# ut-amrl/nautilus

Measured on AMD Instinct MI355X. Metric: loop-closure candidate pairs/sec (1081-beam), higher is better.
Workload: dtype u16

## Files before the change

### nautilus_amd/csm.py

```python
import ctypes as C
import math

import numpy as np

from . import _lib
from ._lib import GridSpec, GridLayout, Search, Match, check, ptr

MATCH_DTYPE = np.dtype([("itheta", "<i4"), ("ix", "<i4"), ("iy", "<i4"), ("score", "<f4")])
assert MATCH_DTYPE.itemsize == C.sizeof(Match) == 16


def grid_spec(range_m=30.0, res=0.05, sigma=2.0, floor_p=1e-10, max_shift=40, cell_bits=16, skip_map=False, no_image=False):
    return GridSpec(float(range_m), float(res), float(sigma), float(floor_p), int(max_shift), int(cell_bits),
                    (_lib.NHIP_GRID_SKIP_MAP if skip_map else 0) | (_lib.NHIP_GRID_NO_IMAGE if no_image else 0), 0)


def search_spec(n_theta=61, nx=81, ny=81, theta_step=math.radians(1.0), exhaustive=False, dense=False, short_scans=False,
                exact_score=False, latency=False):
    flags = (_lib.NHIP_SEARCH_EXHAUSTIVE if exhaustive else 0) | (_lib.NHIP_SEARCH_DENSE if dense else 0) | \
            (_lib.NHIP_SEARCH_SHORT_SCANS if short_scans else 0) | (_lib.NHIP_SEARCH_EXACT_SCORE if exact_score else 0) | \
            (_lib.NHIP_SEARCH_LATENCY if latency else 0)
    return Search(int(n_theta), int(nx), int(ny), flags, float(theta_step))


# ... 175 lines not shown


def gate_floor(spec, min_score, n_points):
    out = C.c_int32(0)
    check(_lib.load().nhip_csm_gate_floor(C.byref(spec), float(min_score), int(n_points), C.byref(out)))
    return out.value


def bnb_stats():
    a, b = C.c_uint64(0), C.c_uint64(0)
    check(_lib.load().nhip_bnb_stats(C.byref(a), C.byref(b)))
    return a.value, b.value


def bnb_stats_levels():
    v = (C.c_uint64 * 24)()
    check(_lib.load().nhip_bnb_stats_levels(v))
    return {"blocks_whole": v[0], "blocks_total": v[1], "candidates_refined": v[2], "sub_blocks": v[3],
            "clk_wave_phase3": v[4], "clk_origins": v[5], "clk_sub_bounds": v[6], "clk_exact": v[7],
            "clk_slowest_wave": v[8], "clk_seeds": v[9], "clk_bounds": v[10], "clk_wave_phase3_100MHz": v[11],
            "pairs_handed_over": v[12], "clk_wave_second_kernel": v[13], "pose_evals16": v[14],
            "pairs_settled_by_gate": v[15], "passes_l2_runs": v[16], "passes_per_cell_field": v[17],
            "passes_per_cell_capacity": v[18], "edge_blocks_refined": v[19], "sub_blocks_without_pose": v[20],
            "edge_blocks_whole": v[21]}


def score_volume(scans, grids, src, slot, theta0, search, origin=(0, 0)):
    out = np.zeros((search.n_theta, search.nx, search.ny), dtype=np.int32)
    check(_lib.load().nhip_csm_scores(scans._h, grids._h, int(src), int(slot), float(theta0),
                                      int(origin[0]), int(origin[1]), C.byref(search), ptr(out)))
    return out


def match_to_transform(m, spec, search, theta0, origin=(0, 0)):
    tx = (origin[0] + int(m["ix"]) - (search.nx - 1) // 2) * spec.res
    ty = (origin[1] + int(m["iy"]) - (search.ny - 1) // 2) * spec.res
    th = theta0 + (int(m["itheta"]) - (search.n_theta - 1) // 2) * search.theta_step
    return np.float32(tx), np.float32(ty), np.float32(th)


class CorrelativeScanMatcher:

    def __init__(self, scanner_range, trans_range, low_res, high_res, sigma=2.0, cell_bits=16):
        self.params = _lib.CsmParams(float(scanner_range), float(trans_range), float(low_res), float(high_res),
                                     float(sigma), 1e-10, int(cell_bits), 0)

    def GetTransformation(self, pointcloud_a, pointcloud_b, rotation_a, rotation_b, rotation_restriction):
        a = np.ascontiguousarray(pointcloud_a, dtype=np.float32).reshape(-1, 2)
        b = np.ascontiguousarray(pointcloud_b, dtype=np.float32).reshape(-1, 2)
        score, tx, ty, th = C.c_double(0), C.c_float(0), C.c_float(0), C.c_float(0)
        check(_lib.load().nhip_csm_get_transformation(C.byref(self.params), ptr(a), len(a), ptr(b), len(b),
                                                      float(rotation_a), float(rotation_b), float(rotation_restriction),
                                                      C.byref(score), C.byref(tx), C.byref(ty), C.byref(th)))
        return score.value, ((np.float32(tx.value), np.float32(ty.value)), np.float32(th.value))


def last_launch():
    out = (C.c_int32 * 8)()
    check(_lib.load().nhip_csm_last_launch(out))
    form = {0: "fused", 1: "split, one round", 2: "split, rounds on one stream", 3: "split, rounds overlapped on the helper stream"}
    return {"form": form.get(out[0], "?"), "form_id": out[0], "pairs_per_round": out[1], "rounds_of_state": out[2],
            "rounds": out[3], "short_scans": bool(out[4]), "hand_over_kernel": bool(out[5]), "instrumented": bool(out[6] & 1),
            "l2_runs": bool(out[6] & 2), "n_pairs": out[7]}


def drop_in_cache_stats():
    v = [C.c_int64(0) for _ in range(4)]
    check(_lib.load().nhip_csm_cache_stats(*[C.byref(x) for x in v]))
    return dict(zip(("entries", "bytes", "hits", "misses"), (x.value for x in v)))


def drop_in_cache_clear():
    check(_lib.load().nhip_csm_cache_clear())


def drop_in_cache_configure(max_bytes):
    check(_lib.load().nhip_csm_cache_configure(int(max_bytes)))
```

### nautilus_amd/csrc/nhip_bnb.hip

```cpp
#include <atomic>
#include <mutex>
#include <type_traits>
#include <vector>

#ifndef NHIP_BNB_INSTR
#define NHIP_BNB_INSTR 0
#endif
#if NHIP_BNB_INSTR
#define csm_bnb_kernel csm_bnb_kernel_instr
#define csm_bnb_rot_kernel csm_bnb_rot_kernel_instr
#define launchers_product launchers_instr
#define BNB_STATS(P) ((P).stats)
#define BNB_TIMELINE(P) ((P).timeline)
#else
#define BNB_STATS(P) (static_cast<unsigned long long *>(nullptr))
#define BNB_TIMELINE(P) (static_cast<unsigned long long *>(nullptr))
#endif

#include "nhip_bnb_params.h"
#include "nhip_bnb_wave.h"
#include "nhip_bnb_origin.h"
#include "nhip_bnb_bounds.h"
#include "nhip_bnb_exact.h"

namespace nhip {

namespace {

using namespace bnb;

constexpr int BNB_THREADS = 64 * BNB_WAVES;

constexpr int N_WORK = 7;
struct PairCtx {
  const uint8_t *grid;
  const float2 *pts;
  int32_t n_pts, cx, cy, pair;
};

template <int CB>
__device__ __forceinline__ void process_candidate(const BnbParams &P, const PairCtx &C, int32_t k, int32_t v, int lane,
                                                  unsigned long long *best, uint32_t (&n)[N_WORK]) {
  const int Y = v / NB, X = v - NB * Y;
  const int32_t vx = block_extent(P.nx, X), vy = block_extent(P.ny, Y);
  const bool edge = vx < BNB_B || vy < BNB_B;
  float cf, sf;
  rotation_k(P, C.pair, k, &cf, &sf);
  if (P.levels >= 2) {
    const __amdgpu_buffer_rsrc_t p4 = uniform_rsrc(C.grid + P.grid_bytes + P.skip_bytes + P.pool_bytes, P.pool4_bytes);
    uint32_t sb[4];
    sub_bounds(P, p4, C.pts, C.n_pts, cf, sf, C.cx, C.cy, Y, X, lane, CB == 1 ? 1u : 257u, sb);
    n[1]++;
    n[4] += edge ? 1u : 0u;
    const uint32_t bsum = best_sum<false>(best);
    int alive = 0;
#pragma unroll
    for (int q = 0; q < 4; q++) alive += (sub_valid(vy, vx, q >> 1, q & 1) && sb[q] != 0u && sb[q] >= bsum) ? 1 : 0;
    if (alive == 0) return;
    if (alive <= 2) {
      const __amdgpu_buffer_rsrc_t rsrc = uniform_rsrc(C.grid, P.grid_bytes + P.skip_bytes);
#pragma unroll 1
      for (int q = 0; q < 4; q++) {
        const uint32_t b = q == 0 ? sb[0] : (q == 1 ? sb[1] : (q == 2 ? sb[2] : sb[3]));
        if (!sub_valid(vy, vx, q >> 1, q & 1) || b == 0u || b < best_sum<false>(best)) continue;
        const unsigned long long key = eval_sub<CB>(P, rsrc, C.pts, C.n_pts, cf, sf, C.cx, C.cy, k, Y, X, q >> 1, q & 1, lane);
        wave_atomic_max(best, key, lane);
        n[2]++;
        n[5] += sub_valid(vy, vx, q >> 1, q & 1) ? 0u : 1u;
      }
      return;
    }
  }
  const unsigned long long key = eval_block<CB>(P, C.grid, C.pts, C.n_pts, cf, sf, C.cx, C.cy, k, Y, X, lane);
  wave_atomic_max(best, key, lane);
  n[0]++;
  n[6] += edge ? 1u : 0u;
}

template <int CB, bool GLOBAL>
__device__ __forceinline__ void process_candidate_c(const BnbParams &P, __amdgpu_buffer_rsrc_t rsrc, uint32_t pitch8,
                                                    __amdgpu_buffer_rsrc_t rsrc16, const uint32_t *org, int32_t nch,
                                                    int32_t n_pts, int32_t k, int32_t Y, int32_t X,
                                                    uint32_t sb0, uint32_t sb1, uint32_t sb2, uint32_t sb3, int lane,
                                                    unsigned long long *best, uint32_t &bcopy, uint32_t (&n)[N_WORK]) {
  const uint32_t bsum = best_sum_cached<GLOBAL>(best, bcopy);
  const int32_t vx = block_extent(P.nx, X), vy = block_extent(P.ny, Y);
  const bool edge = vx < BNB_B || vy < BNB_B;
  n[4] += edge ? 1u : 0u;
  const bool ok0 = sub_valid(vy, vx, 0, 0), ok1 = sub_valid(vy, vx, 0, 1), ok2 = sub_valid(vy, vx, 1, 0), ok3 = sub_valid(vy, vx, 1, 1);
  const int alive = (ok0 && sb0 != 0u && sb0 >= bsum) + (ok1 && sb1 != 0u && sb1 >= bsum) + (ok2 && sb2 != 0u && sb2 >= bsum) +
                    (ok3 && sb3 != 0u && sb3 >= bsum);
  if (alive == 0) return;
  constexpr int WHOLE_MIN = 3;
  if (alive >= WHOLE_MIN) {
    int dy, dx;
    const uint32_t total = block_sums8(rsrc, pitch8, (uint32_t)P.hi_copy_bytes, org, nch, Y, X, lane, &dy, &dx);
    const int32_t ix = BNB_B * X + dx, iy = BNB_B * Y + dy;
    if (CB == 1) {
      const unsigned long long key = best_key(P, k, ix, iy, total, 32);
      wave_atomic_max(best, key, lane);
      if (GLOBAL) bcopy = max(bcopy, (uint32_t)(key >> 32));
    } else {
      n[3] += refine16<GLOBAL>(P, rsrc16, org, nch, n_pts, k, ix, iy, total, true, lane, best, bcopy);
    }
    n[0]++;
    n[6] += __ballot(ix < P.nx && iy < P.ny) != ~0ull ? 1u : 0u;
    return;
  }
#pragma unroll 1
  for (int q = 0; q < 4; q++) {
    const uint32_t b = q == 0 ? sb0 : (q == 1 ? sb1 : (q == 2 ? sb2 : sb3));
    if (!sub_valid(vy, vx, q >> 1, q & 1) || b == 0u || b < best_sum_cached<GLOBAL>(best, bcopy)) continue;
    int dy, dx;
    const uint32_t total = sub_sums8(rsrc, pitch8, (uint32_t)P.hi_copy_bytes, org, nch, Y, X, q >> 1, q & 1, lane, &dy, &dx);
    const int32_t ix = BNB_B * X + BNB_B4 * (q & 1) + dx, iy = BNB_B * Y + BNB_B4 * (q >> 1) + dy;
    if (CB == 1) {
      const unsigned long long key = best_key(P, k, ix, iy, total, 8);
      wave_atomic_max(best, key, lane);
      if (GLOBAL) bcopy = max(bcopy, (uint32_t)(key >> 32));
    } else {
      n[3] += refine16<GLOBAL>(P, rsrc16, org, nch, n_pts, k, ix, iy, total, lane < 16, lane, best, bcopy);
    }
    n[2]++;
    n[5] += __ballot(ix < P.nx && iy < P.ny) == 0ull ? 1u : 0u;
  }
}

struct PhaseClocks {
  long long org, strip, eval;
  uint32_t run_passes, cell_passes_field, cell_passes_full;
};

__device__ __forceinline__ void flush_stats(unsigned long long *stats, const uint32_t *n, int32_t pair, const PhaseClocks *clk,
                                            const uint32_t *edge = nullptr) {
  if (n) {
    if (n[0]) atomicAdd(&stats[0], (unsigned long long)n[0]);
    if (n[1]) atomicAdd(&stats[2], (unsigned long long)n[1]);
    if (n[2]) atomicAdd(&stats[3], (unsigned long long)n[2]);
    if (n[3]) atomicAdd(&stats[14], (unsigned long long)n[3]);
    if (pair < BNB_STATS_PAIRS) atomicAdd(&stats[BNB_STATS_HEAD + pair], 4ull * n[0] + n[2]);
  }
  if (edge) {
    if (edge[0]) atomicAdd(&stats[19], (unsigned long long)edge[0]);
    if (edge[1]) atomicAdd(&stats[20], (unsigned long long)edge[1]);
    if (edge[2]) atomicAdd(&stats[21], (unsigned long long)edge[2]);
  }
  if (clk) {
    atomicAdd(&stats[5], (unsigned long long)clk->org);
    atomicAdd(&stats[6], (unsigned long long)clk->strip);
    atomicAdd(&stats[7], (unsigned long long)clk->eval);
    if (clk->run_passes) atomicAdd(&stats[16], (unsigned long long)clk->run_passes);
    if (clk->cell_passes_field) atomicAdd(&stats[17], (unsigned long long)clk->cell_passes_field);
    if (clk->cell_passes_full) atomicAdd(&stats[18], (unsigned long long)clk->cell_passes_full);
  }
}

template <int CB, bool GLOBAL, bool RUNS = false>
__device__ __forceinline__ void rotation_pass(const BnbParams &P, const PairCtx &C, int32_t k, uint32_t u0, uint32_t u1,
                                              unsigned long long m0, unsigned long long m1, int lane,
                                              unsigned long long *best, uint32_t *done, uint32_t *org,
                                              uint32_t (&n_work)[N_WORK], PhaseClocks &clk, uint32_t *runs = nullptr) {
  long long t_mark = 0;
  float cf, sf;
  rotation_k(P, C.pair, k, &cf, &sf);
  if (BNB_STATS(P)) t_mark = clock64();
  int32_t nrc = RUNS_NONE;
  const int32_t nch = cache_origins<RUNS>(P, C.pts, C.n_pts, cf, sf, C.cx, C.cy, lane, org, true, runs, RUNS && P.l2_runs != 0, &nrc);
  if (BNB_STATS(P)) clk.org += clock64() - t_mark;
  if (RUNS && BNB_STATS(P)) {
    clk.run_passes += nrc > 0 ? 1u : 0u;
    clk.cell_passes_field += nrc == RUNS_FIELD ? 1u : 0u;
    clk.cell_passes_full += nrc == RUNS_FULL ? 1u : 0u;
  }
  const __amdgpu_buffer_rsrc_t rsrc16 = CB == 1 ? uniform_rsrc(C.grid, P.grid_bytes + P.skip_bytes)
                                                : uniform_rsrc(C.grid + P.hi_offset + 2 * P.hi_copy_bytes, P.t16_bytes);
  const __amdgpu_buffer_rsrc_t rsrc = uniform_rsrc(C.grid + P.hi_offset, 2 * P.hi_copy_bytes);
  const uint32_t pitch8 = (uint32_t)P.hi_tpr;
  const __amdgpu_buffer_rsrc_t p4 = uniform_rsrc(C.grid + P.grid_bytes + P.skip_bytes + P.pool_bytes, P.pool4_bytes);
  while ((m0 | m1) != 0ull) {
    const int b0 = m0 ? (int)__builtin_ctzll(m0) : 64 + (int)__builtin_ctzll(m1);
    const int Y = b0 / NB, X0 = b0 - NB * Y;
    int len = 1;
    while (len < 3 && X0 + len < NB) {
      const int b = b0 + len;
      if (!(((b < 64 ? m0 >> b : m1 >> (b - 64)) & 1ull))) break;
      len++;
    }
    uint32_t sb[12];
    uint32_t bcopy = GLOBAL ? best_sum<true>(best) : 0u;
    if (P.levels >= 2) {
      if (BNB_STATS(P)) t_mark = clock64();
      if (RUNS && nrc > 0) strip_bounds_c<RunList<RUN_CHUNKS>>(P, p4, runs + lane, nrc, Y, X0, len, CB == 1 ? 1u : 257u, sb);
      else strip_bounds_c<CellList>(P, p4, org, nch, Y, X0, len, CB == 1 ? 1u : 257u, sb);
      if (BNB_STATS(P)) clk.strip += clock64() - t_mark;
      n_work[1] += (uint32_t)len;
    } else {
#pragma unroll
      for (int q = 0; q < 12; q++) sb[q] = 0xffffffffu;
    }
#pragma unroll 1
    for (int t = 0; t < len; t++) {
      const int b = b0 + t;
      if (b < 64) m0 &= ~(1ull << b);
      else m1 &= ~(1ull << (b - 64));
      const uint32_t ub = (uint32_t)__builtin_amdgcn_readlane((int)(b < 64 ? u0 : u1), b & 63);
      if (ub < best_sum_cached<GLOBAL>(best, bcopy)) continue;
      const uint32_t s0 = t == 0 ? sb[0] : (t == 1 ? sb[4] : sb[8]), s1 = t == 0 ? sb[1] : (t == 1 ? sb[5] : sb[9]);
      const uint32_t s2 = t == 0 ? sb[2] : (t == 1 ? sb[6] : sb[10]), s3 = t == 0 ? sb[3] : (t == 1 ? sb[7] : sb[11]);
      if (BNB_STATS(P)) t_mark = clock64();
      process_candidate_c<CB, GLOBAL>(P, rsrc, pitch8, rsrc16, org, nch, C.n_pts, k, Y, X0 + t, s0, s1, s2, s3, lane, best,
                                      bcopy, n_work);
      if (BNB_STATS(P)) clk.eval += clock64() - t_mark;
      if (done && wave_leader(lane)) done[b] = 0u;
    }
  }
}

__device__ __forceinline__ void read_entry(const RotEntry *ent, int32_t *pair, int32_t *k, unsigned long long *m0,
                                           unsigned long long *m1) {
  const unsigned long long w0 = ent->w[0], w1 = ent->w[1], w2 = ent->w[2], w3 = ent->w[3];
  *pair = (int32_t)(w0 >> 24);
  *k = (int32_t)(w0 & 0xffffffull);
  *m0 = w1 | (w2 << 41);
  *m1 = (w2 >> 23) | (w3 << 18);
}

__device__ __forceinline__ void pair_context(const BnbParams &P, int32_t pair, PairCtx *C) {
  const int32_t src = P.pair_src[pair], slot = P.pair_slot[pair];
  const int32_t beg = P.offsets[src];
  C->grid = P.grids + (size_t)slot * P.slot_bytes;
  C->pts = P.xy + beg;
  C->n_pts = P.offsets[src + 1] - beg;
  C->cx = P.pair_origin ? P.pair_origin[2 * pair] : 0;
  C->cy = P.pair_origin ? P.pair_origin[2 * pair + 1] : 0;
  C->pair = pair;
}
// ... 158 lines not shown
        u1 = s_U[k * 128 + 64 + lane];
        const uint32_t bsum = best_sum<false>(s_best);
        m0 = __ballot(u0 != 0u && u0 >= bsum);
        m1 = __ballot(u1 != 0u && u1 >= bsum && lane + 64 < NB * NB);
        if ((m0 | m1) == 0ull) continue;
        if (heavy && (uint32_t)rank >= P.keep_ranks) {
          const uint32_t lx = (xcd + (uint32_t)rank) & 7u;
          const uint32_t e = wave_fetch_add(P.rot_count + 8 * lx, 1u, lane);
          if (e < P.rot_cap) {
            if (lane < 4) {
              const unsigned long long M41 = (1ull << 41) - 1ull;
              const unsigned long long word = lane == 0   ? ((unsigned long long)(uint32_t)pair << 24) | (uint32_t)k
                                              : lane == 1 ? (m0 & M41)
                                              : lane == 2 ? ((m0 >> 41) | (m1 << 23)) & M41
                                                          : (m1 >> 18);
              P.rot_list[(size_t)lx * P.rot_cap + e].w[lane] = word;
            }
            handed_over = true;
            continue;
          }
        }
        have = true;
      }
      if (have) rotation_pass<CB, false>(P, C, k, u0, u1, m0, m1, lane, s_best, done, org, n_work, clk);
      if (state == SEED) {
        __syncthreads();
        if (BNB_TIMELINE(P) && threadIdx.x == 0 && pair < BNB_STATS_PAIRS) BNB_TIMELINE(P)[4 * pair + 2] = wall_clock64();
        if (BNB_STATS(P)) {
          t_busy = clock64();
          t_wall = wall_clock64();
        }
        for (int32_t kk = threadIdx.x; kk < P.n_theta; kk += THREADS) {
          const unsigned long long mine = s_kmax[kk];
          int32_t rank = 0;
          for (int32_t j = 0; j < P.n_theta; j++) rank += s_kmax[j] > mine ? 1 : 0;
          s_order[rank] = (uint32_t)kk;
        }
        if (P.rot_list || SPLIT) {
          const uint32_t bsum = best_sum<false>(s_best);
          uint32_t mine = 0u;
          for (int32_t kk = wave; kk < P.n_theta; kk += WAVES) {
            const uint32_t c0 = s_U[kk * 128 + lane], c1 = s_U[kk * 128 + 64 + lane];
            mine += (uint32_t)__builtin_popcountll(__ballot(c0 != 0u && c0 >= bsum)) +
                    (uint32_t)__builtin_popcountll(__ballot(c1 != 0u && c1 >= bsum && lane + 64 < NB * NB));
          }
          if (wave_leader(lane)) atomicAdd(s_qn, mine);
        }
// ... 93 lines not shown
    flush_stats(stats_g, nullptr, pair, nullptr, n_work + 4);
  }
  __syncthreads();
  if (threadIdx.x == 0) {
    P.keys[pair] = *s_best;
    if (BNB_TIMELINE(P) && pair < BNB_STATS_PAIRS) {
      uint32_t hw;
      asm volatile("s_getreg_b32 %0, hwreg(HW_REG_HW_ID)" : "=s"(hw));
      uint32_t xcc;
      asm volatile("s_getreg_b32 %0, hwreg(HW_REG_XCC_ID)" : "=s"(xcc));
      BNB_TIMELINE(P)[4 * pair + 3] = (wall_clock64() & 0xfffffffffffull) | ((unsigned long long)((hw >> 8) & 0xffu) << 44) |
                                      ((unsigned long long)(xcc & 0xfu) << 52);
    }
    if (BNB_STATS(P) && BY_ROT) atomicAdd(&BNB_STATS(P)[8], *s_slow);
    if (stats_g) {
      const uint32_t n_all[4] = {s_cnt[0], s_cnt[3], s_cnt[4], s_cnt[5]};
      flush_stats(stats_g, n_all, pair, nullptr);
      atomicAdd(&stats_g[1], (unsigned long long)(P.n_theta * P.nbx * P.nby));
    }
  }
}

template <int CB>
__global__ __launch_bounds__(256, 4) void csm_bnb_rot_kernel(BnbParams P) {
  const int lane = threadIdx.x & 63;
  const uint32_t xcd = blockIdx.x & 7u;
  const uint32_t filled = P.rot_count[8 * xcd];
  const uint32_t count = filled < P.rot_cap ? filled : P.rot_cap;
  const RotEntry *list = P.rot_list + (size_t)xcd * P.rot_cap;
  __shared__ uint32_t s_org2[4 * ORG_WAVE];
  __shared__ uint32_t s_run2[4 * RUN_WAVE];
  uint32_t *org = s_org2 + (threadIdx.x >> 6) * ORG_WAVE + lane;
  uint32_t *runs = s_run2 + (threadIdx.x >> 6) * RUN_WAVE;
  PhaseClocks clk = {0, 0, 0, 0u, 0u, 0u};
  const long long t0 = BNB_STATS(P) ? clock64() : 0;
  for (;;) {
    const uint32_t i = wave_fetch_add(P.rot_count + 8 * xcd + 1, 1u, lane);
    if (i >= count) break;
    int32_t pair, k;
    unsigned long long m0, m1;
    read_entry(list + i, &pair, &k, &m0, &m1);
    PairCtx C;
    pair_context(P, pair, &C);
    uint32_t n[N_WORK] = {};
    rotation_pass<CB, true, true>(P, C, k, 0xffffffffu, 0xffffffffu, m0, m1, lane, &P.keys[pair], nullptr, org, n, clk, runs);
    if (BNB_STATS(P) && lane == 0) flush_stats(BNB_STATS(P), n, pair, nullptr, n + 4);
  }
  if (BNB_STATS(P) && lane == 0) {
    atomicAdd(&BNB_STATS(P)[13], (unsigned long long)(clock64() - t0));
    flush_stats(BNB_STATS(P), nullptr, 0, &clk);
  }
}

constexpr int SORT_THREADS = 1024;
constexpr int SORT_BUCKETS = 16 * 21;
__device__ __forceinline__ int cand_bucket(uint32_t c) {
  if (c == 0u) return SORT_BUCKETS - 1;
  const int e = 31 - __builtin_clz(c);
  const int f = e >= 4 ? (int)((c >> (e - 4)) & 15u) : (int)((c << (4 - e)) & 15u);
  const int b = 16 * e + f;
  return b >= SORT_BUCKETS - 1 ? 0 : SORT_BUCKETS - 2 - b;
}
__device__ __forceinline__ uint32_t cand_shares(const BnbParams &P, uint32_t c) {
  const uint32_t w = 1u + c / P.split_min;
  return w < P.split_max ? w : P.split_max;
}

__global__ __launch_bounds__(SORT_THREADS) void csm_bnb_order_kernel(BnbParams P) {
// ... 94 lines not shown
  }
  __syncthreads();
  unsigned long long *best = shared ? &P.keys[pair] : &s_best2;
  uint32_t *next = shared ? &P.ps_next[pair] : &s_next2;
  const uint32_t *rows = P.ps_rows + (size_t)pair * (size_t)P.n_theta * 128u;
  uint32_t *org = s_org2 + (threadIdx.x >> 6) * ORG_WAVE + lane;
  uint32_t *runs = s_run2 + (threadIdx.x >> 6) * RUN_WAVE;
  PairCtx C;
  pair_context(P, pair, &C);
  uint32_t n_work[N_WORK] = {};
  PhaseClocks clk = {0, 0, 0, 0u, 0u, 0u};
  const long long t0 = BNB_STATS(P) ? clock64() : 0;
  for (;;) {
    const uint32_t rank = wave_fetch_add(next, 1u, lane);
    if (rank >= live) break;
    const uint32_t u0 = rows[(size_t)rank * 128u + lane], u1 = rows[(size_t)rank * 128u + 64 + lane];
    const uint32_t kmax = (uint32_t)__builtin_amdgcn_readlane((int)u1, 62);
    const int32_t k = __builtin_amdgcn_readlane((int)u1, 63);
    const uint32_t bsum = best_sum<true>(best);
    if (kmax < bsum) break;
    const unsigned long long m0 = __ballot(u0 != 0u && u0 >= bsum);
    const unsigned long long m1 = __ballot(u1 != 0u && u1 >= bsum && lane + 64 < NB * NB);
    if ((m0 | m1) == 0ull) continue;
    rotation_pass<CB, true, true>(P, C, k, u0, u1, m0, m1, lane, best, nullptr, org, n_work, clk, runs);
  }
  if (BNB_STATS(P) && lane == 0) {
    atomicAdd(&BNB_STATS(P)[13], (unsigned long long)(clock64() - t0));
    flush_stats(BNB_STATS(P), n_work, pair, &clk, n_work + 4);
  }
  if (BNB_TIMELINE(P) && lane == 0 && pair < BNB_STATS_PAIRS)
    atomicMax(&BNB_TIMELINE(P)[5 * (size_t)BNB_STATS_PAIRS + 2 + pair], wall_clock64());
  if (!shared) {
    __syncthreads();
    if (threadIdx.x == 0) P.keys[pair] = s_best2;
  }
}

}

namespace bnb {

namespace {
template <int CB, bool PL, bool BR, bool SP = false>
int launch_main(const BnbParams &P, const BnbPlan &plan, hipStream_t s) {
  constexpr int THREADS = SP ? 64 * SPLIT_WAVES : BNB_THREADS;
  const size_t lds = lds_bytes((size_t)plan.lds_first, P.n_theta, SP);
  const int64_t blocks = (int64_t)P.pairs_per_xcd * 8;
// ... 74 lines not shown
```

### nautilus_amd/csrc/nhip_bnb_exact.h

```cpp
#pragma once
#include "nhip_bnb_origin.h"

namespace nhip {
namespace {

constexpr int SEG_CHUNKS = 32;
constexpr int EVAL_CHUNKS = 2;

template <bool GLOBAL>
__device__ __forceinline__ uint32_t best_sum(unsigned long long *best) {
  unsigned long long b;
  if (GLOBAL) b = __hip_atomic_load(best, __ATOMIC_RELAXED, __HIP_MEMORY_SCOPE_AGENT);
  else b = *(volatile unsigned long long *)best;
  return (uint32_t)__builtin_amdgcn_readfirstlane((int)(uint32_t)(b >> 32));
}
template <bool GLOBAL>
__device__ __forceinline__ uint32_t best_sum_cached(unsigned long long *best, uint32_t copy) {
  return GLOBAL ? copy : best_sum<false>(best);
}

__device__ __forceinline__ unsigned long long best_key(const BnbParams &P, int32_t k, int32_t ix, int32_t iy, uint32_t total,
                                                       int top) {
  unsigned long long key = 0ull;
  if (ix < P.nx && iy < P.ny) {
// ... 351 lines not shown
    }
  }
  uint32_t R[32];
#pragma unroll
  for (int y = 0; y < 8; y++) {
    R[4 * y + 0] = E[y][0];
    R[4 * y + 1] = O[y][0] - ((E[y][0] >> 16) << 8);
    R[4 * y + 2] = E[y][1];
    R[4 * y + 3] = O[y][1] - ((E[y][1] >> 16) << 8);
  }
  rs_step<32, 1>(R, lane & 1);
  rs_step<16, 2>(R, lane & 2);
  rs_step<8, 4>(R, lane & 4);
  uint32_t V[8];
#pragma unroll
  for (int i = 0; i < 4; i++) {
    V[2 * i] = R[i] & 0xffffu;
    V[2 * i + 1] = R[i] >> 16;
  }
  rs_step<8, 8>(V, lane & 8);
  rs_step<4, 16>(V, lane & 16);
  rs_step<2, 32>(V, lane & 32);
  const int r = 8 * (2 * ((lane >> 5) & 1) + ((lane >> 4) & 1)) + 4 * ((lane >> 2) & 1) + 2 * ((lane >> 1) & 1) + (lane & 1);
  const int f = (lane >> 3) & 1, d = r & 3;
  *dy = r >> 2;
  *dx = 4 * (d >> 1) + (d & 1) + 2 * f;
  return V[0];
}

__device__ __forceinline__ uint32_t pose_sum16(const BnbParams &P, __amdgpu_buffer_rsrc_t rsrc16, const uint32_t *org,
                                               int32_t nch, int32_t ix, int32_t iy) {
  uint32_t acc = 0u;
#pragma unroll
  for (int c = 0; c < OCL; c++) {
    if (c >= nch) continue;
    const uint32_t o = origin_of(org, c);
    acc += org_cnt(o) * (uint32_t)__builtin_amdgcn_raw_buffer_load_b16(
                            rsrc16, (int)t16_tiled(org_row(o) + (uint32_t)iy, org_col(o) + (uint32_t)ix, (uint32_t)P.t16_tpr), 0, 0);
  }
  return wave_sum(acc);
}

template <bool GLOBAL>
__device__ __forceinline__ uint32_t refine16(const BnbParams &P, __amdgpu_buffer_rsrc_t rsrc16, const uint32_t *org,
                                             int32_t nch, int32_t n_pts, int32_t k, int32_t ix, int32_t iy, uint32_t hsum,
                                             bool mine, int lane, unsigned long long *best, uint32_t &bcopy) {
// ... 22 lines not shown
```

### nautilus_amd/csrc/nhip_bnb_host.hip

```cpp
#include <atomic>
#include <memory>
#include <mutex>
#include <vector>

#include "nhip_bnb_params.h"

namespace nhip {

using namespace bnb;

namespace {

size_t bnb_lds_first(const GridLayout &L, bool pool_lds) {
  const size_t pool = pool_lds ? (size_t)L.pool_bytes : 0;
  return pool > (size_t)ORG_LDS ? pool : (size_t)ORG_LDS;
}
size_t bnb_lds_bytes(const GridLayout &L, const nhip_search_t *search, bool pool_lds) {
  return lds_bytes(bnb_lds_first(L, pool_lds), search->n_theta, false);
}
constexpr size_t LDS_MAX = 160 * 1024;

struct TimerScope {
  int id;
  hipStream_t s;
// ... 28 lines not shown
  return BNB_WS_HEADER + 8 * (((n + 7) / 8) * 16 + 64) * (int64_t)sizeof(RotEntry);
}
int64_t bnb_workspace_bytes(int32_t n_pairs) {
  const int64_t n = n_pairs > 0 ? n_pairs : 0;
  nhip_search_t any = {};
  const int64_t m = n <= SPLIT_PAIRS ? n : 2 * SPLIT_PAIRS;
  const int64_t split = bnb_plan(GridLayout(), &any, (int32_t)n, 0).sized_split
                            ? BNB_WS_HEADER + split_state_bytes(m, m / 512 + 4, 64) : 0;
  return std::max(bnb_workspace_bytes_lists(n_pairs), split);
}

BnbPlan bnb_plan(const GridLayout &L, const nhip_search_t *search, int32_t n_pairs, int64_t workspace_bytes) {
  const auto is = [](const char *v, char c) { return v && v[0] == c; };
  const auto num = [](const char *name, int unset) { const char *v = tunable(name); return v ? atoi(v) : unset; };
  const char *force = tunable("NHIP_BNB_KERNELS");
  const char *sp = tunable("NHIP_BNB_SPLIT");
  const char *sbat = tunable("NHIP_BNB_SPLIT_BATCH");
  const char *smax = tunable("NHIP_BNB_SPLIT_MAX");
  BnbPlan p = {};
  p.n_pairs = n_pairs;
  p.cb = L.cb;
  p.levels = is(tunable("NHIP_BNB_LEVELS"), '1') ? 1 : 2;
  p.l2_runs = !is(tunable("NHIP_BNB_L2_RUNS"), '0');
  p.general_all = is(tunable("NHIP_BNB_QUEUE"), '1');
  static_assert(NHIP_SHORT_SCAN_POINTS == 64 * OCL, "the header's promise is the by-rotation form's limit");
  p.short_scans = (search->flags & NHIP_SEARCH_SHORT_SCANS) != 0 && !p.general_all && (uint32_t)(L.S + 2 * L.pad) < ORG_LIMIT;
  p.instrumented = is(tunable("NHIP_BNB_INSTRUMENT"), '1');
  p.stats = p.instrumented && is(tunable("NHIP_BNB_STATS"), '1');
  p.timeline = p.instrumented && is(tunable("NHIP_BNB_TIMELINE"), '1');
  p.sized_split = n_pairs >= SPLIT_MIN_PAIRS || (n_pairs > 0 && (is(sp, '1') || sbat));
  if (workspace_bytes > 0 && n_pairs > 0 && !p.general_all && !is(sp, '0') && !is(force, '2') &&
      (n_pairs >= SPLIT_MIN_PAIRS || is(sp, '1'))) {
    p.batch = sbat && atoi(sbat) > 0 ? atoi(sbat) : SPLIT_PAIRS;
    if (p.batch > n_pairs) p.batch = n_pairs;
    for (;;) {
      p.slot_bytes = (split_state_bytes(p.batch, 1, search->n_theta) + 511) & ~(int64_t)511;
      p.slots = (workspace_bytes - BNB_WS_HEADER - 512) / p.slot_bytes;
      const int64_t rounds = (n_pairs + p.batch - 1) / p.batch;
      if (p.slots >= (rounds < 2 ? rounds : 2) || p.batch <= 512) break;
      p.batch = p.batch / 2 > 512 ? p.batch / 2 : 512;
    }
    if (p.slots > SPLIT_RING) p.slots = SPLIT_RING;
    if (p.slots < 1) p.batch = 0;
    if (!sbat && p.batch > 0 && n_pairs > p.batch && (p.slots < 2 || p.batch < SPLIT_PAIRS)) p.batch = 0;
  }
  p.rounds = p.batch > 0 ? (n_pairs + p.batch - 1) / p.batch : 1;
// ... 37 lines not shown
  n->device = dev;
  hipError_t e = hipStreamCreateWithFlags(&n->stream, hipStreamNonBlocking);
  for (int i = 0; i < SPLIT_RING && e == hipSuccess; i++) {
    e = hipEventCreateWithFlags(&n->ea[i], hipEventDisableTiming);
    if (e == hipSuccess) e = hipEventCreateWithFlags(&n->eb[i], hipEventDisableTiming);
  }
  if (e != hipSuccess) {
    delete n;
    return hip_fail(e, "split form: helper stream / events", __FILE__, __LINE__);
  }
  *out = n;
  return NHIP_OK;
}
static void split_set_release(SplitSet *set) {
  if (!set) return;
  std::lock_guard<std::mutex> lock(g_split_mu);
  g_split_free.push_back(set);
}

static thread_local BnbPlan t_last_plan = {};
void bnb_last_launch(int32_t out[8]) {
  const BnbPlan &p = t_last_plan;
  const int32_t info[8] = {p.form, (int32_t)p.batch, (int32_t)p.slots, (int32_t)p.rounds, p.short_scans, p.second,
                           (int32_t)p.instrumented | ((int32_t)p.l2_runs << 1), p.n_pairs};
  memcpy(out, info, sizeof(info));
}

static void fill_bnb_params(BnbParams &P, const MatchJob &job, const BnbPlan &plan) {
  const GridLayout &L = *job.L;
  fill_job_params(P, job);
  P.pair_kbase = job.pair_kbase;
  P.keys = reinterpret_cast<unsigned long long *>(job.keys);
  P.gate = job_gate(job);
  P.nbx = (P.nx + BNB_B - 1) / BNB_B;
  P.nby = (P.ny + BNB_B - 1) / BNB_B;
  P.pool_pitch = L.pool_pitch;
  P.pool_rows = L.pool_rows;
  P.pairs_per_xcd = (plan.n_pairs + 7) / 8;
  P.skip_bytes = L.skip_bytes;
  P.pool_bytes = L.pool_bytes;
  P.pool4_bytes = L.pool4_bytes;
  P.pool4_pitch = L.pool4_pitch;
  P.hi_offset = L.hi_offset;
  P.hi_bytes = L.hi_bytes;
  P.hi_pitch = L.hi_pitch;
  P.hi_tpr = L.hi_tpr;
  P.hi_copy_bytes = L.hi_copy_bytes;
  P.t16_bytes = L.t16_bytes;
  P.t16_tpr = L.t16_tpr;
  P.inv_res_f = (float)P.inv_res;
  P.levels = plan.levels;
  P.l2_runs = plan.l2_runs;
  P.general_all = plan.general_all;
  P.short_scans = plan.short_scans;
  P.heavy_min = plan.heavy_min;
  P.keep_ranks = plan.keep_ranks;
  P.rot_cap = plan.rot_cap;
  P.lds_first = (int32_t)plan.lds_first;
}

static int instr_buffers(const BnbPlan &plan, BnbParams &P, hipStream_t s) {
  if (!plan.stats && !plan.timeline) return NHIP_OK;
  std::lock_guard<std::mutex> lock(g_instr_mu);
  if (plan.stats) {
    if (!g_bnb_stats) {
      NHIP_TRY_HIP(hipMalloc(reinterpret_cast<void **>(&g_bnb_stats), 8 * (BNB_STATS_HEAD + (size_t)BNB_STATS_PAIRS)));
      NHIP_TRY_HIP(hipMemset(g_bnb_stats, 0, 8 * (BNB_STATS_HEAD + (size_t)BNB_STATS_PAIRS)));
    }
    P.stats = g_bnb_stats;
  }
  if (plan.timeline) {
    if (!g_bnb_timeline) NHIP_TRY_HIP(hipMalloc(reinterpret_cast<void **>(&g_bnb_timeline), 48 * (size_t)BNB_STATS_PAIRS + 16));
    P.timeline = g_bnb_timeline;
    NHIP_TRY_HIP(hipMemsetAsync(g_bnb_timeline + 4 * (size_t)BNB_STATS_PAIRS + 2, 0xff, 8 * (size_t)BNB_STATS_PAIRS, s));
    NHIP_TRY_HIP(hipMemsetAsync(g_bnb_timeline + 5 * (size_t)BNB_STATS_PAIRS + 2, 0, 8 * (size_t)BNB_STATS_PAIRS, s));
// ... 135 lines not shown
```

### nautilus_amd/csrc/nhip_bnb_params.h

```cpp
#pragma once
#include "nhip_common.h"
#include "nhip_csm_shared.h"

namespace nhip {
namespace bnb {

constexpr int BNB_WAVES = 8;
constexpr int NB = BNB_MAX_NB;
constexpr int MAX_ROT = 340;
constexpr int QCAP = 1024;
constexpr int SPLIT_WAVES = 8;
constexpr int LIST_ENTRIES = 128;
constexpr int RUN_SHIFT = 25;
constexpr int OC = 18;
constexpr int OCL = 17;
constexpr int ORG_WAVE = OCL * 64;
constexpr int ORG_LDS = BNB_WAVES * ORG_WAVE * 4;
constexpr uint32_t ORG_LIMIT = 1u << 13;
constexpr int RUN_CHUNKS = 8;
constexpr int RUN_WAVE = RUN_CHUNKS * 64;

constexpr int QSPACE_SPLIT = (SPLIT_WAVES * LIST_ENTRIES * 4 + MAX_ROT * 12 + 15) / 16 * 2;
constexpr int lds_qspace(bool split) { return split ? QSPACE_SPLIT : QCAP; }
static_assert(QSPACE_SPLIT <= QCAP, "the split form's LDS must not exceed the fused form's, which bnb_fits() checks");
// ... 46 lines not shown
  uint32_t split_min;
  uint32_t split_max;
  uint32_t front_min;
  int32_t pair_base;
  int32_t n_pairs, n_theta, nx, ny, hx, hy, nbx, nby;
  int32_t S, pad, pitch, rows, max_shift;
  int32_t pool_pitch, pool_rows, pairs_per_xcd;
  int32_t pool4_pitch;
  int32_t lds_first;
  int32_t general_all;
  int32_t short_scans;
  int32_t levels;
  int64_t grid_bytes, skip_bytes, slot_bytes, pool_bytes, pool4_bytes;
  int64_t hi_offset, hi_bytes;
  int32_t hi_pitch;
  int32_t hi_tpr;
  int64_t hi_copy_bytes;
  int64_t t16_bytes;
  int32_t t16_tpr;
  double res, inv_res;
  float inv_res_f;
  ScoreGate gate;
  int32_t l2_runs;
};

using BnbLaunch = int (*)(const BnbParams &P, const BnbPlan &plan, hipStream_t s);
struct BnbLaunchers { BnbLaunch fused, split_a, split_b; };
BnbLaunchers launchers_product();
BnbLaunchers launchers_instr();

}
}
```

### nautilus_amd/csrc/nhip_common.h

```cpp
#pragma once
#include <hip/hip_runtime.h>

#include <cmath>
#include <cstdint>
#include <cstdio>
#include <cstring>
#include <string>
#include <vector>

#include "../../include/nautilus_hip_debug.h"

namespace nhip {

void set_error(const char *fmt, ...);
int hip_fail(hipError_t e, const char *what, const char *file, int line);

#define NHIP_TRY_HIP(expr)                                            \
  do {                                                                \
    hipError_t _e = (expr);                                           \
    if (_e != hipSuccess) return ::nhip::hip_fail(_e, #expr, __FILE__, __LINE__); \
  } while (0)

#define NHIP_REQUIRE(cond, ...)          \
  do {                                   \
// ... 125 lines not shown
int launch_grid_build(const float *d_xy, const int32_t *d_offsets, int32_t n_scans, const int32_t *d_target_ids,
                      int32_t n_targets, const nhip_grid_spec_t *spec, const GridLayout &L,
                      uint8_t *d_grids, void *d_ws, int64_t ws_bytes, hipStream_t s, bool incremental = false);

enum MatchForm : int32_t {
  MATCH_BNB,
  MATCH_POSES,
  MATCH_STRIPS8,
  MATCH_STRIPS16,
};
struct MatchPlan {
  MatchForm form = MATCH_BNB;
  int32_t tile_rows = 0, n_tiles = 0;
  bool keys_zeroed = false, keys_undecoded = false;
};
MatchPlan csm_plan(const GridLayout &L, const nhip_search_t *search, int32_t n_pairs);

enum BnbForm : int32_t { BNB_FUSED, BNB_SPLIT_ONE, BNB_SPLIT_ROUNDS, BNB_SPLIT_OVERLAP };
struct BnbPlan {
  BnbForm form;
  int32_t n_pairs, cb, levels;
  bool second, general_all, short_scans, pool_lds, instrumented, stats, timeline;
  bool l2_runs;
  bool sized_split;
  uint32_t rot_cap, heavy_min, keep_ranks, split_min, split_max;
  int64_t batch, slots, slot_bytes, rounds;
  int64_t lds_first;
};
BnbPlan bnb_plan(const GridLayout &L, const nhip_search_t *search, int32_t n_pairs, int64_t workspace_bytes);

struct MatchJob {
  const float *xy = nullptr;
  const int32_t *offsets = nullptr;
  IdBounds ids = {0, 0, nullptr};
  const uint8_t *grids = nullptr;
  const nhip_grid_spec_t *spec = nullptr;
  const GridLayout *L = nullptr;
  const int32_t *pair_src = nullptr, *pair_slot = nullptr;
  const double *rot0_cs = nullptr;
  const double *delta_cs = nullptr;
  const int32_t *pair_origin = nullptr, *pair_kbase = nullptr;
  int32_t n_pairs = 0;
  const nhip_search_t *search = nullptr;
  double min_score = -INFINITY;
  uint64_t *keys = nullptr;
  nhip_match_t *out = nullptr;
// ... 268 lines not shown
```

Baseline: 1.771 million.

## Evaluate adjacent surviving sub-blocks in pairs across a strip in the rotation kernel

In the by-rotation kernel path, surviving sub-blocks are no longer evaluated inside each block's candidate loop. Their masks are collected across the strip, and horizontally adjacent survivors are then scored together with a new pair_sums8 that loads 12-byte rows and reduces both halves in one pass. The intent is to cut redundant grid loads and reductions and to keep more lanes busy per evaluation. The kernel's launch bounds for CB==2 also rise from 4 to 5 blocks per CU, which adds register pressure and risks spills.

```diff
diff --git a/nautilus_amd/csm.py b/nautilus_amd/csm.py
--- a/nautilus_amd/csm.py
+++ b/nautilus_amd/csm.py
@@ -221,7 +221,7 @@
             "pairs_handed_over": v[12], "clk_wave_second_kernel": v[13], "pose_evals16": v[14],
             "pairs_settled_by_gate": v[15], "passes_l2_runs": v[16], "passes_per_cell_field": v[17],
             "passes_per_cell_capacity": v[18], "edge_blocks_refined": v[19], "sub_blocks_without_pose": v[20],
-            "edge_blocks_whole": v[21]}
+            "edge_blocks_whole": v[21], "pair_passes": v[22], "pair_passes_across_blocks": v[23]}
 
 
 def score_volume(scans, grids, src, slot, theta0, search, origin=(0, 0)):
@@ -260,7 +260,7 @@
     form = {0: "fused", 1: "split, one round", 2: "split, rounds on one stream", 3: "split, rounds overlapped on the helper stream"}
     return {"form": form.get(out[0], "?"), "form_id": out[0], "pairs_per_round": out[1], "rounds_of_state": out[2],
             "rounds": out[3], "short_scans": bool(out[4]), "hand_over_kernel": bool(out[5]), "instrumented": bool(out[6] & 1),
-            "l2_runs": bool(out[6] & 2), "n_pairs": out[7]}
+            "l2_runs": bool(out[6] & 2), "pair_subs": bool(out[6] & 4), "n_pairs": out[7]}
 
 
 def drop_in_cache_stats():
diff --git a/nautilus_amd/csrc/nhip_bnb.hip b/nautilus_amd/csrc/nhip_bnb.hip
--- a/nautilus_amd/csrc/nhip_bnb.hip
+++ b/nautilus_amd/csrc/nhip_bnb.hip
@@ -31,7 +31,7 @@
 
 constexpr int BNB_THREADS = 64 * BNB_WAVES;
 
-constexpr int N_WORK = 7;
+constexpr int N_WORK = 9;
 struct PairCtx {
   const uint8_t *grid;
   const float2 *pts;
@@ -77,12 +77,13 @@
   n[6] += edge ? 1u : 0u;
 }
 
-template <int CB, bool GLOBAL>
+template <int CB, bool GLOBAL, bool PAIR>
 __device__ __forceinline__ void process_candidate_c(const BnbParams &P, __amdgpu_buffer_rsrc_t rsrc, uint32_t pitch8,
                                                     __amdgpu_buffer_rsrc_t rsrc16, const uint32_t *org, int32_t nch,
                                                     int32_t n_pts, int32_t k, int32_t Y, int32_t X,
                                                     uint32_t sb0, uint32_t sb1, uint32_t sb2, uint32_t sb3, int lane,
-                                                    unsigned long long *best, uint32_t &bcopy, uint32_t (&n)[N_WORK]) {
+                                                    unsigned long long *best, uint32_t &bcopy, uint32_t (&n)[N_WORK],
+                                                    int t, uint32_t &mk0, uint32_t &mk1) {
   const uint32_t bsum = best_sum_cached<GLOBAL>(best, bcopy);
   const int32_t vx = block_extent(P.nx, X), vy = block_extent(P.ny, Y);
   const bool edge = vx < BNB_B || vy < BNB_B;
@@ -107,22 +108,85 @@
     n[6] += __ballot(ix < P.nx && iy < P.ny) != ~0ull ? 1u : 0u;
     return;
   }
+  if (!PAIR) {
 #pragma unroll 1
-  for (int q = 0; q < 4; q++) {
-    const uint32_t b = q == 0 ? sb0 : (q == 1 ? sb1 : (q == 2 ? sb2 : sb3));
-    if (!sub_valid(vy, vx, q >> 1, q & 1) || b == 0u || b < best_sum_cached<GLOBAL>(best, bcopy)) continue;
-    int dy, dx;
-    const uint32_t total = sub_sums8(rsrc, pitch8, (uint32_t)P.hi_copy_bytes, org, nch, Y, X, q >> 1, q & 1, lane, &dy, &dx);
-    const int32_t ix = BNB_B * X + BNB_B4 * (q & 1) + dx, iy = BNB_B * Y + BNB_B4 * (q >> 1) + dy;
-    if (CB == 1) {
-      const unsigned long long key = best_key(P, k, ix, iy, total, 8);
-      wave_atomic_max(best, key, lane);
-      if (GLOBAL) bcopy = max(bcopy, (uint32_t)(key >> 32));
-    } else {
-      n[3] += refine16<GLOBAL>(P, rsrc16, org, nch, n_pts, k, ix, iy, total, lane < 16, lane, best, bcopy);
-    }
-    n[2]++;
-    n[5] += __ballot(ix < P.nx && iy < P.ny) == 0ull ? 1u : 0u;
+    for (int q = 0; q < 4; q++) {
+      const uint32_t b = q == 0 ? sb0 : (q == 1 ? sb1 : (q == 2 ? sb2 : sb3));
+      if (!sub_valid(vy, vx, q >> 1, q & 1) || b == 0u || b < best_sum_cached<GLOBAL>(best, bcopy)) continue;
+      int dy, dx;
+      const uint32_t total = sub_sums8(rsrc, pitch8, (uint32_t)P.hi_copy_bytes, org, nch, Y, X, q >> 1, q & 1, lane, &dy, &dx);
+      const int32_t ix = BNB_B * X + BNB_B4 * (q & 1) + dx, iy = BNB_B * Y + BNB_B4 * (q >> 1) + dy;
+      if (CB == 1) {
+        const unsigned long long key = best_key(P, k, ix, iy, total, 8);
+        wave_atomic_max(best, key, lane);
+        if (GLOBAL) bcopy = max(bcopy, (uint32_t)(key >> 32));
+      } else {
+        n[3] += refine16<GLOBAL>(P, rsrc16, org, nch, n_pts, k, ix, iy, total, lane < 16, lane, best, bcopy);
+      }
+      n[2]++;
+      n[5] += __ballot(ix < P.nx && iy < P.ny) == 0ull ? 1u : 0u;
+    }
+    return;
+  }
+  mk0 |= (uint32_t)((ok0 && sb0 != 0u && sb0 >= bsum) | ((ok1 && sb1 != 0u && sb1 >= bsum) << 1)) << (2 * t);
+  mk1 |= (uint32_t)((ok2 && sb2 != 0u && sb2 >= bsum) | ((ok3 && sb3 != 0u && sb3 >= bsum) << 1)) << (2 * t);
+}
+
+#ifndef NHIP_BNB_PAIR_CROSS
+#define NHIP_BNB_PAIR_CROSS 0
+#endif
+constexpr bool PAIR_CROSS = NHIP_BNB_PAIR_CROSS != 0;
+__device__ __forceinline__ uint32_t pick6(const uint32_t (&r)[6], int c) {
+  return c == 0 ? r[0] : (c == 1 ? r[1] : (c == 2 ? r[2] : (c == 3 ? r[3] : (c == 4 ? r[4] : r[5]))));
+}
+template <int CB, bool GLOBAL>
+__device__ __forceinline__ void strip_sub_blocks(const BnbParams &P, __amdgpu_buffer_rsrc_t rsrc, uint32_t pitch8,
+                                                 __amdgpu_buffer_rsrc_t rsrc16, const uint32_t *org, int32_t nch, int32_t n_pts,
+                                                 int32_t k, int32_t Y, int32_t X0, const uint32_t (&sb)[12], uint32_t mk0,
+                                                 uint32_t mk1, int lane, unsigned long long *best, uint32_t &bcopy,
+                                                 uint32_t (&n)[N_WORK]) {
+#pragma unroll 1
+  for (int sy = 0; sy < 2; sy++) {
+    uint32_t mk = sy ? mk1 : mk0;
+    if (mk == 0u) continue;
+    uint32_t row[6];
+#pragma unroll
+    for (int c = 0; c < 6; c++) row[c] = sy ? sb[4 * (c >> 1) + 2 + (c & 1)] : sb[4 * (c >> 1) + (c & 1)];
+#pragma unroll 1
+    while (mk != 0u) {
+      const int c = (int)__builtin_ctz(mk);
+      mk &= mk - 1u;
+      const uint32_t bsum = best_sum_cached<GLOBAL>(best, bcopy);
+      if (pick6(row, c) < bsum) continue;
+      const int32_t X = X0 + (c >> 1), sx = c & 1;
+      const bool two = P.pair_subs != 0 && ((mk >> (c + 1)) & 1u) != 0u && (PAIR_CROSS || sx == 0) && pick6(row, c + 1) >= bsum;
+      int dy, dx;
+      uint32_t total;
+      if (two) {
+        mk &= ~(1u << (c + 1));
+        total = pair_sums8(rsrc, pitch8, (uint32_t)P.hi_copy_bytes, org, nch, Y, X, sy, sx, lane, &dy, &dx);
+      } else {
+        total = sub_sums8(rsrc, pitch8, (uint32_t)P.hi_copy_bytes, org, nch, Y, X, sy, sx, lane, &dy, &dx);
+      }
+      const int32_t ix = BNB_B * X + BNB_B4 * sx + dx, iy = BNB_B * Y + BNB_B4 * sy + dy;
+      if (CB == 1) {
+        const unsigned long long key = best_key(P, k, ix, iy, total, 16);
+        wave_atomic_max(best, key, lane);
+        if (GLOBAL) bcopy = max(bcopy, (uint32_t)(key >> 32));
+      } else {
+        n[3] += refine16<GLOBAL>(P, rsrc16, org, nch, n_pts, k, ix, iy, total, lane < (two ? 32 : 16), lane, best, bcopy);
+      }
+      const bool pose = ix < P.nx && iy < P.ny;
+      if (two) {
+        n[2] += 2u;
+        n[5] += (__ballot(pose && dx < BNB_B4) == 0ull ? 1u : 0u) + (__ballot(pose && dx >= BNB_B4) == 0ull ? 1u : 0u);
+        n[7]++;
+        n[8] += (uint32_t)sx;
+      } else {
+        n[2]++;
+        n[5] += __ballot(pose) == 0ull ? 1u : 0u;
+      }
+    }
   }
 }
 
@@ -144,6 +208,8 @@
     if (edge[0]) atomicAdd(&stats[19], (unsigned long long)edge[0]);
     if (edge[1]) atomicAdd(&stats[20], (unsigned long long)edge[1]);
     if (edge[2]) atomicAdd(&stats[21], (unsigned long long)edge[2]);
+    if (edge[3]) atomicAdd(&stats[22], (unsigned long long)edge[3]);
+    if (edge[4]) atomicAdd(&stats[23], (unsigned long long)edge[4]);
   }
   if (clk) {
     atomicAdd(&stats[5], (unsigned long long)clk->org);
@@ -155,7 +221,7 @@
   }
 }
 
-template <int CB, bool GLOBAL, bool RUNS = false>
+template <int CB, bool GLOBAL, bool PAIR, bool RUNS = false>
 __device__ __forceinline__ void rotation_pass(const BnbParams &P, const PairCtx &C, int32_t k, uint32_t u0, uint32_t u1,
                                               unsigned long long m0, unsigned long long m1, int lane,
                                               unsigned long long *best, uint32_t *done, uint32_t *org,
@@ -198,6 +264,7 @@
 #pragma unroll
       for (int q = 0; q < 12; q++) sb[q] = 0xffffffffu;
     }
+    uint32_t mk0 = 0u, mk1 = 0u;
 #pragma unroll 1
     for (int t = 0; t < len; t++) {
       const int b = b0 + t;
@@ -208,10 +275,15 @@
       const uint32_t s0 = t == 0 ? sb[0] : (t == 1 ? sb[4] : sb[8]), s1 = t == 0 ? sb[1] : (t == 1 ? sb[5] : sb[9]);
       const uint32_t s2 = t == 0 ? sb[2] : (t == 1 ? sb[6] : sb[10]), s3 = t == 0 ? sb[3] : (t == 1 ? sb[7] : sb[11]);
       if (BNB_STATS(P)) t_mark = clock64();
-      process_candidate_c<CB, GLOBAL>(P, rsrc, pitch8, rsrc16, org, nch, C.n_pts, k, Y, X0 + t, s0, s1, s2, s3, lane, best,
-                                      bcopy, n_work);
+      process_candidate_c<CB, GLOBAL, PAIR>(P, rsrc, pitch8, rsrc16, org, nch, C.n_pts, k, Y, X0 + t, s0, s1, s2, s3, lane, best,
+                                      bcopy, n_work, t, mk0, mk1);
       if (BNB_STATS(P)) clk.eval += clock64() - t_mark;
       if (done && wave_leader(lane)) done[b] = 0u;
+    }
+    if (PAIR && (mk0 | mk1) != 0u) {
+      if (BNB_STATS(P)) t_mark = clock64();
+      strip_sub_blocks<CB, GLOBAL>(P, rsrc, pitch8, rsrc16, org, nch, C.n_pts, k, Y, X0, sb, mk0, mk1, lane, best, bcopy, n_work);
+      if (BNB_STATS(P)) clk.eval += clock64() - t_mark;
     }
   }
 }
@@ -416,7 +488,7 @@
         }
         have = true;
       }
-      if (have) rotation_pass<CB, false>(P, C, k, u0, u1, m0, m1, lane, s_best, done, org, n_work, clk);
+      if (have) rotation_pass<CB, false, false>(P, C, k, u0, u1, m0, m1, lane, s_best, done, org, n_work, clk);
       if (state == SEED) {
         __syncthreads();
         if (BNB_TIMELINE(P) && threadIdx.x == 0 && pair < BNB_STATS_PAIRS) BNB_TIMELINE(P)[4 * pair + 2] = wall_clock64();
@@ -556,7 +628,7 @@
 }
 
 template <int CB>
-__global__ __launch_bounds__(256, 4) void csm_bnb_rot_kernel(BnbParams P) {
+__global__ __launch_bounds__(256, CB == 2 && !NHIP_BNB_INSTR ? 5 : 4) void csm_bnb_rot_kernel(BnbParams P) {
   const int lane = threadIdx.x & 63;
   const uint32_t xcd = blockIdx.x & 7u;
   const uint32_t filled = P.rot_count[8 * xcd];
@@ -577,7 +649,7 @@
     PairCtx C;
     pair_context(P, pair, &C);
     uint32_t n[N_WORK] = {};
-    rotation_pass<CB, true, true>(P, C, k, 0xffffffffu, 0xffffffffu, m0, m1, lane, &P.keys[pair], nullptr, org, n, clk, runs);
+    rotation_pass<CB, true, true, true>(P, C, k, 0xffffffffu, 0xffffffffu, m0, m1, lane, &P.keys[pair], nullptr, org, n, clk, runs);
     if (BNB_STATS(P) && lane == 0) flush_stats(BNB_STATS(P), n, pair, nullptr, n + 4);
   }
   if (BNB_STATS(P) && lane == 0) {
@@ -718,7 +790,7 @@
     const unsigned long long m0 = __ballot(u0 != 0u && u0 >= bsum);
     const unsigned long long m1 = __ballot(u1 != 0u && u1 >= bsum && lane + 64 < NB * NB);
     if ((m0 | m1) == 0ull) continue;
-    rotation_pass<CB, true, true>(P, C, k, u0, u1, m0, m1, lane, best, nullptr, org, n_work, clk, runs);
+    rotation_pass<CB, true, true, true>(P, C, k, u0, u1, m0, m1, lane, best, nullptr, org, n_work, clk, runs);
   }
   if (BNB_STATS(P) && lane == 0) {
     atomicAdd(&BNB_STATS(P)[13], (unsigned long long)(clock64() - t0));
diff --git a/nautilus_amd/csrc/nhip_bnb_exact.h b/nautilus_amd/csrc/nhip_bnb_exact.h
--- a/nautilus_amd/csrc/nhip_bnb_exact.h
+++ b/nautilus_amd/csrc/nhip_bnb_exact.h
@@ -397,6 +397,56 @@
   rs_step<4, 16>(V, lane & 16);
   rs_step<2, 32>(V, lane & 32);
   const int r = 8 * (2 * ((lane >> 5) & 1) + ((lane >> 4) & 1)) + 4 * ((lane >> 2) & 1) + 2 * ((lane >> 1) & 1) + (lane & 1);
+  const int f = (lane >> 3) & 1, d = r & 3;
+  *dy = r >> 2;
+  *dx = 4 * (d >> 1) + (d & 1) + 2 * f;
+  return V[0];
+}
+
+__device__ __forceinline__ uint32_t pair_sums8(__amdgpu_buffer_rsrc_t rsrc, uint32_t pitch, uint32_t copy_bytes, const uint32_t *org,
+                                               int32_t nch, int32_t Y, int32_t X, int32_t sy, int32_t sx0, int lane, int *dy, int *dx) {
+  const uint32_t roff = (uint32_t)(BNB_B * Y + BNB_B4 * sy), coff = (uint32_t)(BNB_B * X + BNB_B4 * sx0);
+  const uint32_t wrap = pitch * HI_TILE_BYTES - HI_TILE_BYTES;
+  static_assert(257u * 255u <= 0xffffu, "a packed field holds the byte sums of the 8 lanes it is reduced over");
+  uint32_t E[4][2], O[4][2];
+#pragma unroll
+  for (int y = 0; y < 4; y++) E[y][0] = E[y][1] = O[y][0] = O[y][1] = 0u;
+#pragma unroll
+  for (int r = 0; r < OC; r++) {
+    if (r >= nch) continue;
+    const uint32_t o = origin_of(org, r);
+    const uint32_t cn = org_cnt(o);
+    const uint32_t row0 = org_row(o) + roff, col0 = org_col(o) + coff, col4 = col0 & ~3u;
+    const uint32_t q = row0 & 7u, sh = (col0 & 3u) * 8u;
+    const uint32_t g = hi_tiled(row0, col4, (col4 >> 3) & 1u, pitch, copy_bytes);
+    u32x3 w[4];
+#pragma unroll
+    for (int y = 0; y < 4; y++)
+      w[y] = __builtin_amdgcn_raw_buffer_load_b96(rsrc, (int)(g + (q + (uint32_t)y >= 8u ? wrap : 0u) + 16u * (uint32_t)y), 0, 0);
+#pragma unroll
+    for (int y = 0; y < 4; y++) {
+      const uint32_t n0 = __builtin_amdgcn_alignbit(w[y].y, w[y].x, sh);
+      const uint32_t n1 = __builtin_amdgcn_alignbit(w[y].z, w[y].y, sh);
+      E[y][0] += __umul24(n0 & M8, cn); O[y][0] += __umul24(n0 >> 8, cn);
+      E[y][1] += __umul24(n1 & M8, cn); O[y][1] += __umul24(n1 >> 8, cn);
+    }
+  }
+  uint32_t R[16];
+#pragma unroll
+  for (int y = 0; y < 4; y++) {
+    R[4 * y + 0] = E[y][0];
+    R[4 * y + 1] = O[y][0] - ((E[y][0] >> 16) << 8);
+    R[4 * y + 2] = E[y][1];
+    R[4 * y + 3] = O[y][1] - ((E[y][1] >> 16) << 8);
+  }
+  rs_step<16, 1>(R, lane & 1);
+  rs_step<8, 2>(R, lane & 2);
+  rs_step<4, 4>(R, lane & 4);
+  uint32_t V[4] = {R[0] & 0xffffu, R[0] >> 16, R[1] & 0xffffu, R[1] >> 16};
+  rs_step<4, 8>(V, lane & 8);
+  rs_step<2, 16>(V, lane & 16);
+  V[0] = add_xor<32>(V[0]);
+  const int r = 8 * ((lane >> 4) & 1) + 4 * ((lane >> 2) & 1) + 2 * ((lane >> 1) & 1) + (lane & 1);
   const int f = (lane >> 3) & 1, d = r & 3;
   *dy = r >> 2;
   *dx = 4 * (d >> 1) + (d & 1) + 2 * f;
diff --git a/nautilus_amd/csrc/nhip_bnb_host.hip b/nautilus_amd/csrc/nhip_bnb_host.hip
--- a/nautilus_amd/csrc/nhip_bnb_host.hip
+++ b/nautilus_amd/csrc/nhip_bnb_host.hip
@@ -74,6 +74,7 @@
   p.cb = L.cb;
   p.levels = is(tunable("NHIP_BNB_LEVELS"), '1') ? 1 : 2;
   p.l2_runs = !is(tunable("NHIP_BNB_L2_RUNS"), '0');
+  p.pair_subs = !is(tunable("NHIP_BNB_PAIR_SUBS"), '0');
   p.general_all = is(tunable("NHIP_BNB_QUEUE"), '1');
   static_assert(NHIP_SHORT_SCAN_POINTS == 64 * OCL, "the header's promise is the by-rotation form's limit");
   p.short_scans = (search->flags & NHIP_SEARCH_SHORT_SCANS) != 0 && !p.general_all && (uint32_t)(L.S + 2 * L.pad) < ORG_LIMIT;
@@ -157,7 +158,7 @@
 void bnb_last_launch(int32_t out[8]) {
   const BnbPlan &p = t_last_plan;
   const int32_t info[8] = {p.form, (int32_t)p.batch, (int32_t)p.slots, (int32_t)p.rounds, p.short_scans, p.second,
-                           (int32_t)p.instrumented | ((int32_t)p.l2_runs << 1), p.n_pairs};
+                           (int32_t)p.instrumented | ((int32_t)p.l2_runs << 1) | ((int32_t)p.pair_subs << 2), p.n_pairs};
   memcpy(out, info, sizeof(info));
 }
 
@@ -186,6 +187,7 @@
   P.inv_res_f = (float)P.inv_res;
   P.levels = plan.levels;
   P.l2_runs = plan.l2_runs;
+  P.pair_subs = plan.pair_subs;
   P.general_all = plan.general_all;
   P.short_scans = plan.short_scans;
   P.heavy_min = plan.heavy_min;
diff --git a/nautilus_amd/csrc/nhip_bnb_params.h b/nautilus_amd/csrc/nhip_bnb_params.h
--- a/nautilus_amd/csrc/nhip_bnb_params.h
+++ b/nautilus_amd/csrc/nhip_bnb_params.h
@@ -92,6 +92,7 @@
   float inv_res_f;
   ScoreGate gate;
   int32_t l2_runs;
+  int32_t pair_subs;
 };
 
 using BnbLaunch = int (*)(const BnbParams &P, const BnbPlan &plan, hipStream_t s);
diff --git a/nautilus_amd/csrc/nhip_common.h b/nautilus_amd/csrc/nhip_common.h
--- a/nautilus_amd/csrc/nhip_common.h
+++ b/nautilus_amd/csrc/nhip_common.h
@@ -171,6 +171,7 @@
   int32_t n_pairs, cb, levels;
   bool second, general_all, short_scans, pool_lds, instrumented, stats, timeline;
   bool l2_runs;
+  bool pair_subs;
   bool sized_split;
   uint32_t rot_cap, heavy_min, keep_ranks, split_min, split_max;
   int64_t batch, slots, slot_bytes, rounds;
```

Measured after the change: 1.822 million, median of 6. 1.03x the previous value.
